# TEAM-AIOLY/OCM-VAE-SIMCA

Hardware: AMD Instinct MI355X
Metric: spectra/sec SIMCA fit+Q/T² score at 1M×2048 (higher is better)
Workload: dtype f32

## Files before the change

### ocm-vae-simca_amd/csrc/ocm_score.hip

```cpp
#include "ocm_internal.h"

#include <utility>

namespace {

constexpr int SW = 4;
constexpr int SR = 32;
constexpr int SROWS = SW * SR;

struct DecArgs {
  int32_t enabled;
  int32_t type;
  double t2_scale, q_scale, dlim;
};

using ocm::dred_of;

template <int KT, int NW>
__device__ __forceinline__ void score_epilogue(double* tls, double* sred, const double (&accT64)[KT][16], double q64,
                                               int64_t row0, int64_t m, int k, int a_diag,
                                               const double* __restrict__ A, float* __restrict__ T_out,
                                               double* T2_out, float* __restrict__ Q_out, DecArgs dec,
                                               double* __restrict__ acc_out, int64_t acc_stride,
                                               double* __restrict__ stat_part, int ldt = 0,
// ... 261 lines not shown
template <int N>
__device__ __forceinline__ void wait_vv(f32x4& h) {
  asm volatile("s_waitcnt vmcnt(%1)" : "+v"(h) : "n"(N));
}
__device__ __forceinline__ float xlane(int src, float v) {
  return __builtin_bit_cast(float, __builtin_amdgcn_ds_bpermute(src, __builtin_bit_cast(int, v)));
}

#ifdef OCM_S1P_DIAG_NOMFMA
#define OCM_MF(ACC, A, B) ""
#define OCM_M4(ACC, A, B) ""
#else
#define OCM_MF(ACC, A, B) "v_mfma_f32_16x16x4_f32 %[" #ACC "], %[" #A "], %[" #B "], %[" #ACC "]\n\t"
#define OCM_M4(ACC, A, B) "v_mfma_f32_4x4x1_16b_f32 %[" #ACC "], %[" #A "], %[" #B "], %[" #ACC "]\n\t"
#endif
template <bool EX>
__device__ __forceinline__ void s1_block(f32x4& acA, f32x4& acB, f32x4& acC, f32x4& acD, f32x4& acE, f32x4& acF,
                                         const f32x4& a, const float (&b)[4], const f32x4& x) {
  if constexpr (EX)
    asm("s_nop 1\n\t" OCM_M4(cE, b0, x0) OCM_MF(cA, a0, x0) OCM_M4(cF, b1, x1) OCM_MF(cB, a1, x1)
            OCM_M4(cE, b2, x2) OCM_MF(cC, a2, x2) OCM_M4(cF, b3, x3) OCM_MF(cD, a3, x3)
        : [cA] "+v"(acA), [cB] "+v"(acB), [cC] "+v"(acC), [cD] "+v"(acD), [cE] "+v"(acE), [cF] "+v"(acF)
        : [a0] "v"(a[0]), [a1] "v"(a[1]), [a2] "v"(a[2]), [a3] "v"(a[3]), [b0] "v"(b[0]), [b1] "v"(b[1]),
          [b2] "v"(b[2]), [b3] "v"(b[3]), [x0] "a"(x[0]), [x1] "a"(x[1]), [x2] "a"(x[2]), [x3] "a"(x[3]));
  else
    asm("s_nop 1\n\t" OCM_MF(cA, a0, x0) OCM_MF(cB, a1, x1) OCM_MF(cC, a2, x2) OCM_MF(cD, a3, x3)
        : [cA] "+v"(acA), [cB] "+v"(acB), [cC] "+v"(acC), [cD] "+v"(acD)
        : [a0] "v"(a[0]), [a1] "v"(a[1]), [a2] "v"(a[2]), [a3] "v"(a[3]), [x0] "a"(x[0]), [x1] "a"(x[1]),
          [x2] "a"(x[2]), [x3] "a"(x[3]));
}

#ifdef OCM_S1P_DIAG_NOMFMA
#define OCM_M2(R, A, T) ""
#else
#define OCM_M2(R, A, T) "v_mfma_f32_16x16x4_f32 %[" #R "], %[" #A "], %[" #T "], %[" #R "]\n\t"
#endif
#define OCM_RD(S, P) "v_accvgpr_read_b32 %[" #S "], %[" #P "]\n\t"
#define OCM_FM(Q, S) "v_fmac_f32_e32 %[" #Q "], %[" #S "], %[" #S "]\n\t"
template <bool EX, bool QW>
__device__ __forceinline__ void s2_pair(f32x4& x0, f32x4& x1, const float (&a0)[5], const float (&a1)[5], float m0,
                                        float m1, const float (&tB)[5], float one, const f32x4& p0, const f32x4& p1,
                                        float (&q)[4]) {
  float s[4];
  if constexpr (EX && QW)
    asm volatile("s_nop 1\n\t" OCM_M4(x0, m0, on) OCM_M4(x1, m1, on) "s_nop 4\n\t" OCM_M2(x0, u0, t0) OCM_M2(x1, w0, t0) OCM_RD(s0, p00) OCM_RD(s1, p10) OCM_RD(s2, p01) OCM_RD(s3, p11) OCM_M2(x0, u1, t1) OCM_FM(q0, s0) OCM_FM(q1, s1) OCM_FM(q2, s2) OCM_FM(q3, s3) OCM_M2(x1, w1, t1) OCM_RD(s0, p02) OCM_RD(s1, p12) OCM_RD(s2, p03) OCM_RD(s3, p13) OCM_M2(x0, u2, t2) OCM_FM(q0, s0) OCM_FM(q1, s1) OCM_FM(q2, s2) OCM_FM(q3, s3) OCM_M2(x1, w2, t2) OCM_M2(x0, u3, t3) OCM_M2(x1, w3, t3) OCM_M2(x0, u4, t4) OCM_M2(x1, w4, t4)
        : [x0] "+a"(x0), [x1] "+a"(x1), [q0] "+v"(q[0]), [q1] "+v"(q[1]), [q2] "+v"(q[2]), [q3] "+v"(q[3]), [s0] "=&v"(s[0]), [s1] "=&v"(s[1]), [s2] "=&v"(s[2]), [s3] "=&v"(s[3])
        : [u0] "v"(a0[0]), [u1] "v"(a0[1]), [u2] "v"(a0[2]), [u3] "v"(a0[3]), [u4] "v"(a0[4]), [w0] "v"(a1[0]), [w1] "v"(a1[1]), [w2] "v"(a1[2]), [w3] "v"(a1[3]), [w4] "v"(a1[4]), [m0] "v"(m0), [m1] "v"(m1), [t0] "v"(tB[0]), [t1] "v"(tB[1]), [t2] "v"(tB[2]), [t3] "v"(tB[3]), [t4] "v"(tB[4]), [on] "v"(one), [p00] "a"(p0[0]), [p01] "a"(p0[1]), [p02] "a"(p0[2]), [p03] "a"(p0[3]), [p10] "a"(p1[0]), [p11] "a"(p1[1]), [p12] "a"(p1[2]), [p13] "a"(p1[3]));
  else if constexpr (EX)
    asm volatile("s_nop 1\n\t" OCM_M4(x0, m0, on) OCM_M4(x1, m1, on) "s_nop 4\n\t" OCM_M2(x0, u0, t0) OCM_M2(x1, w0, t0) OCM_M2(x0, u1, t1) OCM_M2(x1, w1, t1) OCM_M2(x0, u2, t2) OCM_M2(x1, w2, t2) OCM_M2(x0, u3, t3) OCM_M2(x1, w3, t3) OCM_M2(x0, u4, t4) OCM_M2(x1, w4, t4)
        : [x0] "+a"(x0), [x1] "+a"(x1)
        : [u0] "v"(a0[0]), [u1] "v"(a0[1]), [u2] "v"(a0[2]), [u3] "v"(a0[3]), [u4] "v"(a0[4]), [w0] "v"(a1[0]), [w1] "v"(a1[1]), [w2] "v"(a1[2]), [w3] "v"(a1[3]), [w4] "v"(a1[4]), [m0] "v"(m0), [m1] "v"(m1), [t0] "v"(tB[0]), [t1] "v"(tB[1]), [t2] "v"(tB[2]), [t3] "v"(tB[3]), [t4] "v"(tB[4]), [on] "v"(one));
  else if constexpr (QW)
    asm volatile("s_nop 1\n\t" OCM_M4(x0, m0, on) OCM_M4(x1, m1, on) "s_nop 4\n\t" OCM_M2(x0, u0, t0) OCM_M2(x1, w0, t0) OCM_RD(s0, p00) OCM_RD(s1, p10) OCM_RD(s2, p01) OCM_RD(s3, p11) OCM_M2(x0, u1, t1) OCM_FM(q0, s0) OCM_FM(q1, s1) OCM_FM(q2, s2) OCM_FM(q3, s3) OCM_M2(x1, w1, t1) OCM_RD(s0, p02) OCM_RD(s1, p12) OCM_RD(s2, p03) OCM_RD(s3, p13) OCM_M2(x0, u2, t2) OCM_FM(q0, s0) OCM_FM(q1, s1) OCM_FM(q2, s2) OCM_FM(q3, s3) OCM_M2(x1, w2, t2) OCM_M2(x0, u3, t3) OCM_M2(x1, w3, t3)
        : [x0] "+a"(x0), [x1] "+a"(x1), [q0] "+v"(q[0]), [q1] "+v"(q[1]), [q2] "+v"(q[2]), [q3] "+v"(q[3]), [s0] "=&v"(s[0]), [s1] "=&v"(s[1]), [s2] "=&v"(s[2]), [s3] "=&v"(s[3])
        : [u0] "v"(a0[0]), [u1] "v"(a0[1]), [u2] "v"(a0[2]), [u3] "v"(a0[3]), [w0] "v"(a1[0]), [w1] "v"(a1[1]), [w2] "v"(a1[2]), [w3] "v"(a1[3]), [m0] "v"(m0), [m1] "v"(m1), [t0] "v"(tB[0]), [t1] "v"(tB[1]), [t2] "v"(tB[2]), [t3] "v"(tB[3]), [on] "v"(one), [p00] "a"(p0[0]), [p01] "a"(p0[1]), [p02] "a"(p0[2]), [p03] "a"(p0[3]), [p10] "a"(p1[0]), [p11] "a"(p1[1]), [p12] "a"(p1[2]), [p13] "a"(p1[3]));
  else
    asm volatile("s_nop 1\n\t" OCM_M4(x0, m0, on) OCM_M4(x1, m1, on) "s_nop 4\n\t" OCM_M2(x0, u0, t0) OCM_M2(x1, w0, t0) OCM_M2(x0, u1, t1) OCM_M2(x1, w1, t1) OCM_M2(x0, u2, t2) OCM_M2(x1, w2, t2) OCM_M2(x0, u3, t3) OCM_M2(x1, w3, t3)
        : [x0] "+a"(x0), [x1] "+a"(x1)
        : [u0] "v"(a0[0]), [u1] "v"(a0[1]), [u2] "v"(a0[2]), [u3] "v"(a0[3]), [w0] "v"(a1[0]), [w1] "v"(a1[1]), [w2] "v"(a1[2]), [w3] "v"(a1[3]), [m0] "v"(m0), [m1] "v"(m1), [t0] "v"(tB[0]), [t1] "v"(tB[1]), [t2] "v"(tB[2]), [t3] "v"(tB[3]), [on] "v"(one));
  (void)s, (void)p0, (void)p1, (void)q;
}
template <bool EX>
__device__ __forceinline__ void s1_block_v(f32x4& acA, f32x4& acB, f32x4& acC, f32x4& acD, f32x4& acE, f32x4& acF,
                                           const f32x4& a, const float (&b)[4], const f32x4& x) {
  if constexpr (EX)
    asm("s_nop 1\n\t" OCM_M4(cE, b0, x0) OCM_MF(cA, a0, x0) OCM_M4(cF, b1, x1) OCM_MF(cB, a1, x1)
            OCM_M4(cE, b2, x2) OCM_MF(cC, a2, x2) OCM_M4(cF, b3, x3) OCM_MF(cD, a3, x3)
        : [cA] "+v"(acA), [cB] "+v"(acB), [cC] "+v"(acC), [cD] "+v"(acD), [cE] "+v"(acE), [cF] "+v"(acF)
        : [a0] "v"(a[0]), [a1] "v"(a[1]), [a2] "v"(a[2]), [a3] "v"(a[3]), [b0] "v"(b[0]), [b1] "v"(b[1]),
          [b2] "v"(b[2]), [b3] "v"(b[3]), [x0] "v"(x[0]), [x1] "v"(x[1]), [x2] "v"(x[2]), [x3] "v"(x[3]));
  else
    asm("s_nop 1\n\t" OCM_MF(cA, a0, x0) OCM_MF(cB, a1, x1) OCM_MF(cC, a2, x2) OCM_MF(cD, a3, x3)
        : [cA] "+v"(acA), [cB] "+v"(acB), [cC] "+v"(acC), [cD] "+v"(acD)
        : [a0] "v"(a[0]), [a1] "v"(a[1]), [a2] "v"(a[2]), [a3] "v"(a[3]), [x0] "v"(x[0]), [x1] "v"(x[1]),
          [x2] "v"(x[2]), [x3] "v"(x[3]));
}
#undef OCM_MF
#undef OCM_M4
#undef OCM_M2
#undef OCM_RD
#undef OCM_FM
}

#ifdef OCM_S1P_W8
static bool s1p_w8_enabled() {
  const char* v = getenv("OCM_S1P_W8_ON");
  return !v || v[0] != '0';
}
#endif

template <int NJ, bool EX, int HH = -1, int WV = 4>
__global__ __launch_bounds__(64 * WV, 1) void k_score_1p(const float* __restrict__ X, int64_t ldx,
                                                     const int64_t* __restrict__ rows, int64_t m,
                                                     const double* __restrict__ P, const double* __restrict__ mu,
                                                     const double* __restrict__ adiag, int k,
                                                     float* __restrict__ T_out, double* __restrict__ T2_out,
                                                     float* __restrict__ Q_out, DecArgs dec,
                                                     double* __restrict__ acc_out, int64_t acc_stride,
                                                     double* __restrict__ stat_part, int64_t ntiles,
                                                     PrepArgs pa, const float* __restrict__ ptaps,
                                                     const float* __restrict__ prow) {
  using namespace s1p;
  constexpr int W = WV;
  constexpr int NT = 64 * WV;
  constexpr int TPB = WV == 4 ? 2 : 1;
  constexpr bool PREP = HH >= 0;
  constexpr int GL = NJ + (HH > 0 ? 1 : 0);
  constexpr int PW = 16 * NJ;
  constexpr int PP = W * PW;
  constexpr int NCH = PP / 4;
  static_assert(NJ % 4 == 0 && 2 * NJ - 1 <= 63, "64-column wave slices, vmcnt range");
  __shared__ f32x4 P0s[16 * NCH];
  __shared__ float nmuL[PP];
  __shared__ double pmuL[20];
  __shared__ double tpart[TPB][W * 20 * R];
  __shared__ double qpart[2][W * R];
  const int tid = threadIdx.x, lane = tid & 63;
  const int w = __builtin_amdgcn_readfirstlane(tid >> 6);
  const int ln = lane & 15, lq = lane >> 4;

  {
    constexpr int PE = 16 * NCH / NT;
    constexpr int UB = PE < 8 ? PE : 8;
    static_assert(PE % UB == 0, "prologue batches");
#pragma unroll
    for (int i0 = 0; i0 < PE; i0 += UB) {
      double v[UB][4];
#pragma unroll
      for (int u = 0; u < UB; ++u) {
        const int e = tid + (i0 + u) * NT, c = e / NCH, ch = e - c * NCH;
        const double* src = P + (int64_t)(c < k ? c : 0) * PP + 4 * ch;
#pragma unroll
        for (int q = 0; q < 4; ++q) v[u][q] = src[q];
      }
#pragma unroll
      for (int u = 0; u < UB; ++u) {
        const int e = tid + (i0 + u) * NT, c = e / NCH, ch = e - c * NCH;
        f32x4 x;
#pragma unroll
        for (int q = 0; q < 4; ++q) x[q] = c < k ? (float)v[u][q] : 0.f;
        P0s[c * NCH + (ch ^ sw(c))] = x;
      }
    }
    constexpr int ME = PP / NT;
    float nm[ME];
#pragma unroll
    for (int i = 0; i < ME; ++i) nm[i] = -(float)mu[tid + i * NT];
#pragma unroll
    for (int i = 0; i < ME; ++i) nmuL[tid + i * NT] = nm[i];
    constexpr int CL = PP / 64;
    double muv[CL];
#pragma unroll
    for (int i = 0; i < CL; ++i) muv[i] = mu[lane + 64 * i];
    for (int c = w; c < 20; c += W) {
      double s = 0.0;
      if (c < k) {
        double pv[CL];
#pragma unroll
        for (int i = 0; i < CL; ++i) pv[i] = P[(int64_t)c * PP + lane + 64 * i];
#pragma unroll
        for (int i = 0; i < CL; ++i) s += pv[i] * muv[i];
      }
      s = wave_sum_f64(s);
      if (lane == 0) pmuL[c] = s;
    }
  }
  float p1a[EX ? NJ : 1];
  constexpr bool NOP1B = EX && ((NJ == 32 && HH > 4) || WV == 8);
  float p1b[EX && !NOP1B ? NJ : 1];
  if constexpr (EX) {
    const bool p1v = 16 + lq < k;
    const double* p1r = P + (int64_t)(p1v ? 16 + lq : 0) * PP + w * PW;
    double pa_[NJ], pb_[NOP1B ? 1 : NJ];
#pragma unroll
    for (int j = 0; j < NJ; ++j) {
      pa_[j] = p1r[16 * j + ln];
      if constexpr (!NOP1B) pb_[j] = p1r[16 * j + (ln ^ (8 * (lq >> 1)))];
    }
#pragma unroll
    for (int j = 0; j < NJ; ++j) {
      p1a[j] = p1v ? (float)pa_[j] : 0.f;
      if constexpr (!NOP1B) p1b[j] = p1v ? (float)pb_[j] : 0.f;
    }
  }
  __shared__ double adL[WV == 8 ? 20 : 1];
  double ad[WV == 8 ? 1 : 5];
  if constexpr (WV == 8) {
    if (tid < 20) adL[tid] = tid < k ? adiag[tid] : 0.0;
  } else {
#pragma unroll
    for (int s = 0; s < 5; ++s) ad[s] = lq + 4 * s < k ? adiag[lq + 4 * s] : 0.0;
  }
  int b1[4];
#pragma unroll
  for (int b = 0; b < 4; ++b) b1[b] = ln * NCH + w * (PW / 4) + ((4 * b + lq) ^ sw(ln));
  int b2[4][4];
#pragma unroll
  for (int s = 0; s < 4; ++s)
#pragma unroll
    for (int b = 0; b < 4; ++b) {
      const int c = 4 * s + lq;
      b2[s][b] = 4 * (c * NCH + w * (PW / 4) + ((4 * b + (ln >> 2)) ^ sw(c))) + (ln & 3);
    }
  const float* p0f = reinterpret_cast<const float*>(P0s);
  const int bperm = 4 * (16 * (ln & 3) + ((4 * lq) ^ (8 * ((ln & 3) >> 1))));
  const int bpermA = 4 * (16 * (ln & 3) + 4 * lq);
  const float one = 1.f;
  __syncthreads();

  const int64_t G = gridDim.x;
  auto col_base = [&](int64_t row) { return X + row * ldx + w * PW + 4 * lq; };
  auto index_of = [&](int64_t tt) -> int64_t {
    if (!rows) {
      const int64_t r = tt * R + ln;
      return r < m ? r : m - 1;
    }
    int64_t v = 0;
#pragma unroll
    for (int i = 0; i < R; ++i) {
      const int64_t r = tt * R + i;
      const int64_t ri = rows[r < m ? r : m - 1];
      v = ln == i ? ri : v;
    }
    return v;
  };

  f32x4 XA[NJ], XB[NJ];
  double st[4] = {0.0, 0.0, 0.0, 0.0};
  double tt[5];
  float tB[5];
  double T2 = 0.0, T2prev = 0.0;

  float ctap[HH > 0 ? HH + 1 : 1];
  if constexpr (HH > 0)
#pragma unroll
    for (int t = 1; t <= HH; ++t) ctap[t] = ptaps[HH + t];
  auto rowstat_of = [&](int64_t tt, float& mr, float& sr) {
    mr = 0.f;
    sr = 1.f;
    if (!PREP || !pa.snv) return;
#pragma unroll
    for (int i = 0; i < R; ++i) {
      const int64_t r = tt * R + i;
      const int64_t rr = r < m ? r : m - 1;
      const int64_t xi = rows ? rows[rr] : rr;
      const float mi = prow[2 * xi], si = prow[2 * xi + 1];
      mr = ln == i ? mi : mr;
      sr = ln == i ? si : sr;
    }
  };
  auto stencil_e = [&](const float* win, float sr, int e) __attribute__((always_inline)) -> float {
    const int o = (HH > 0 ? HH : 0) + e;
    float a;
    if constexpr (HH <= 0) {
      a = win[o];
    } else {
      a = 0.f;
#pragma unroll
      for (int t = 1; t <= HH; ++t) a = fmaf(ctap[t], __fsub_rn(win[o + t], win[o - t]), a);
    }
    return ocm::mul_nc(a, sr);
  };
  auto stencil = [&](const float* win, float sr) __attribute__((always_inline)) -> f32x4 {
    f32x4 y;
#pragma unroll
    for (int e = 0; e < 4; ++e) y[e] = stencil_e(win, sr, e);
    return y;
  };
  auto edge_fix = [&](f32x4& y, const f32x4& ucur, float sr, bool left) __attribute__((always_inline)) {
    if constexpr (HH > 0) {
      f32x4 q1, q2, q3;
#pragma unroll
      for (int e = 0; e < 4; ++e) {
        q1[e] = xlane(4 * (lane ^ 16), ucur[e]);
        q2[e] = xlane(4 * (lane ^ 32), ucur[e]);
        q3[e] = xlane(4 * (lane ^ 48), ucur[e]);
      }
      float row16[16];
#pragma unroll
      for (int sq = 0; sq < 4; ++sq)
#pragma unroll
        for (int e = 0; e < 4; ++e) {
          const int kk = lq ^ sq;
          row16[4 * sq + e] = kk == 0 ? ucur[e] : kk == 1 ? q1[e] : kk == 2 ? q2[e] : q3[e];
        }
      const int Wn = 2 * HH + 1;
#pragma unroll
      for (int i = 0; i < HH; ++i) {
        const float* et = ptaps + Wn + (left ? i : HH + i) * Wn;
        const int s0 = left ? 0 : 16 - Wn;
        const int cl = left ? i : 16 - HH + i;
        const float ref = row16[cl];
        float a = 0.f;
#pragma unroll
        for (int t = 0; t < Wn; ++t) a = fmaf(et[t], __fsub_rn(row16[s0 + t], ref), a);
        const float yv = ocm::mul_nc(a, sr);
#pragma unroll
        for (int e = 0; e < 4; ++e)
          if (4 * lq + e == cl) y[e] = yv;
      }
    }
  };

  auto exchange = [&](const f32x4& uprev, const f32x4& ucur, const f32x4& unext, float* win)
      __attribute__((always_inline)) {
    constexpr int H_ = HH > 0 ? HH : 0;
    constexpr int NL1 = H_ < 4 ? H_ : 4;
#pragma unroll
    for (int e = 4 - NL1; e < 4; ++e) {
      win[H_ - 4 + e] = xlane(4 * ((lane + 48) & 63), lq == 3 ? uprev[e] : ucur[e]);
      win[H_ + 4 + (e - (4 - NL1))] =
          xlane(4 * ((lane + 16) & 63), lq == 0 ? unext[e - (4 - NL1)] : ucur[e - (4 - NL1)]);
    }
    if constexpr (H_ > 4) {
#pragma unroll
      for (int e = 8 - H_; e < 4; ++e)
        win[H_ - 8 + e] = xlane(4 * (lane ^ 32), lq >= 2 ? uprev[e] : ucur[e]);
#pragma unroll
      for (int e = 0; e < H_ - 4; ++e)
        win[H_ + 8 + e] = xlane(4 * (lane ^ 32), lq <= 1 ? unext[e] : ucur[e]);
    }
#pragma unroll
    for (int e = 0; e < 4; ++e) win[H_ + e] = ucur[e];
  };

  auto sweep1 = [&](f32x4 (&Y)[NJ], f32x4& hy, int buf, int64_t tile, auto XGc) __attribute__((always_inline)) {
    constexpr int XG = decltype(XGc)::value;
    f32x4 acA = {0.f, 0.f, 0.f, 0.f}, acB = acA, acC = acA, acD = acA, acE = acA, acF = acA;
    double t64[4] = {0.0, 0.0, 0.0, 0.0}, x164[4] = {0.0, 0.0, 0.0, 0.0};
    f32x4 aN = P0s[b1[0]];
    float bN[4] = {0.f, 0.f, 0.f, 0.f};
    if constexpr (EX)
#pragma unroll
      for (int e = 0; e < 4; ++e)
        bN[e] = NOP1B ? xlane(bpermA + 4 * e, p1a[0])
                      : __builtin_bit_cast(float, __builtin_amdgcn_ds_bpermute(bperm + 4 * e, __builtin_bit_cast(int, p1b[0])));
    auto operands = [&](auto J, f32x4& a, float (&b)[4]) __attribute__((always_inline)) {
      constexpr int j = decltype(J)::value;
      a = aN;
#pragma unroll
      for (int e = 0; e < 4; ++e) b[e] = bN[e];
      if constexpr (j + 1 < NJ) {
        aN = P0s[b1[(j + 1) & 3] + 16 * ((j + 1) >> 2)];
        if constexpr (EX)
#pragma unroll
          for (int e = 0; e < 4; ++e)
            bN[e] = __builtin_bit_cast(float,
                                       __builtin_amdgcn_ds_bpermute(NOP1B ? bpermA + 4 * e : bperm + 4 * e,
                                                                    __builtin_bit_cast(int, NOP1B ? p1a[j + 1] : p1b[NOP1B ? 0 : j + 1])));
      }
    };
    auto flush = [&]() __attribute__((always_inline)) {
      asm volatile("s_nop 11" : "+v"(acA), "+v"(acB), "+v"(acC), "+v"(acD), "+v"(acE), "+v"(acF));
#pragma unroll
      for (int i = 0; i < 4; ++i) {
        t64[i] += ((double)acA[i] + (double)acB[i]) + ((double)acC[i] + (double)acD[i]);
        x164[i] += (double)acE[i] + (double)acF[i];
        acA[i] = acB[i] = acC[i] = acD[i] = acE[i] = acF[i] = 0.f;
      }
    };
    if constexpr (!PREP) {
      static_for<NJ>([&](auto J) {
        constexpr int j = decltype(J)::value;
        f32x4 a;
        float b[4];
        operands(J, a, b);
        wait_vm<NJ - 1 - j + XG>(Y[j]);
        s1_block<EX>(acA, acB, acC, acD, acE, acF, a, b, Y[j]);
        __builtin_amdgcn_sched_barrier(0);
        if constexpr ((j & 15) == 15 || j == NJ - 1) {
          flush();
        }
      });
    } else {
      constexpr int H_ = HH > 0 ? HH : 0;
      float win[4 + 2 * H_];
      float mr, sr;
      rowstat_of(tile, mr, sr);
      constexpr int W0 = NJ - 3 + XG < 63 ? NJ - 3 + XG : 63;
      wait_vm<W0>(Y[2]);
      wait_vm<W0>(Y[1]);
      wait_vm<W0>(Y[0]);
      wait_vv<W0>(hy);
      auto raw = [&](const f32x4& v) __attribute__((always_inline)) {
        f32x4 u = v;
        if constexpr (HH == 0)
#pragma unroll
          for (int e = 0; e < 4; ++e) u[e] = __fsub_rn(u[e], mr);
        return u;
      };
      f32x4 uprev = raw(hy), ucur = raw(Y[0]), unext = raw(Y[1]);
      f32x4 yE = {0.f, 0.f, 0.f, 0.f};
      if constexpr (HH > 0) {
        wait_vm<XG>(Y[NJ - 1]);
        if (w == 0) edge_fix(yE, ucur, sr, true);
        if (w == W - 1) edge_fix(yE, raw(Y[NJ - 1]), sr, false);
      }
      auto patch = [&](f32x4& y, bool right) __attribute__((always_inline)) {
        if constexpr (HH > 0)
#pragma unroll
          for (int e = 0; e < 4; ++e) {
            const int cl = 4 * lq + e;
            const bool ed = right ? (w == W - 1) & (cl >= 16 - HH) : (w == 0) & (cl < HH);
            y[e] = ed ? yE[e] : y[e];
          }
      };
      auto advance = [&](const f32x4& nx) __attribute__((always_inline)) {
        unext = raw(nx);
        exchange(uprev, ucur, unext, win);
        uprev = ucur;
        ucur = unext;
      };
      exchange(uprev, ucur, unext, win);
      uprev = ucur;
      ucur = unext;
      f32x4 y = stencil(win, sr);
      patch(y, false);
      if constexpr (NJ == 1) patch(y, true);
      advance(Y[2]);
      static_for<NJ>([&](auto J) {
        constexpr int j = decltype(J)::value;
        f32x4 a;
        float b[4];
        operands(J, a, b);
        f32x4 yn = y;
#pragma unroll
        for (int e = 0; e < 4; ++e) {
          if constexpr (EX)
            (e & 1 ? acF : acE) = __builtin_amdgcn_mfma_f32_4x4x1f32(b[e], y[e], e & 1 ? acF : acE, 0, 0, 0);
          f32x4& c = e == 0 ? acA : e == 1 ? acB : e == 2 ? acC : acD;
          c = __builtin_amdgcn_mfma_f32_16x16x4f32(a[e], y[e], c, 0, 0, 0);
          if constexpr (j + 1 < NJ) yn[e] = stencil_e(win, sr, e);
        }
        asm volatile("" : "=a"(Y[j]) : "0"(y));
        if constexpr (j + 1 < NJ) {
          y = yn;
          if constexpr (j + 1 == NJ - 1) patch(y, true);
          if constexpr (j + 2 < NJ) {
            if constexpr (j + 3 < NJ) {
              wait_vm<NJ - 4 - j + XG>(Y[j + 3]);
              advance(Y[j + 3]);
            } else {
              advance(hy);
            }
          }
        }
        __builtin_amdgcn_sched_barrier(0);
        if constexpr ((j & 15) == 15 || j == NJ - 1) {
          flush();
        }
      });
    }
    if constexpr (TPB == 1) {
      asm volatile("s_waitcnt lgkmcnt(0)" ::: "memory");
      __builtin_amdgcn_s_barrier();
      asm volatile("" ::: "memory");
    }
    double* tp = tpart[TPB == 1 ? 0 : buf];
#pragma unroll
    for (int i = 0; i < 4; ++i) tp[(w * 20 + 4 * lq + i) * R + ln] = t64[i];
    if constexpr (EX) {
#pragma unroll
      for (int u = 0; u < 4; ++u) {
        x164[u] += __shfl_xor(x164[u], 16, 64);
        x164[u] += __shfl_xor(x164[u], 32, 64);
      }
      if (lq == 0)
#pragma unroll
        for (int u = 0; u < 4; ++u) tp[(w * 20 + 16 + u) * R + ln] = x164[u];
    }
  };
  auto compute_t = [&](int64_t t, int buf) {
    const double* tp = tpart[TPB == 1 ? 0 : buf];
#pragma unroll
    for (int s = 0; s < 5; ++s) {
      double v = 0.0;
      if (s < 4 || EX) {
#pragma unroll
        for (int ww = 0; ww < W; ++ww) v += tp[(ww * 20 + lq + 4 * s) * R + ln];
        v -= pmuL[lq + 4 * s];
      }
      tt[s] = v;
    }
    T2 = 0.0;
#pragma unroll
    for (int s = 0; s < 5; ++s) T2 += tt[s] * tt[s] * (WV == 8 ? adL[lq + 4 * s] : ad[s < (WV == 8 ? 1 : 5) ? s : 0]);
    T2 += __shfl_xor(T2, 16, 64);
    T2 += __shfl_xor(T2, 32, 64);
    const int64_t row = t * R + ln;
    if (T_out && w == 0 && row < m)
#pragma unroll
      for (int s = 0; s < 5; ++s)
        if (lq + 4 * s < k) T_out[row * k + lq + 4 * s] = (float)tt[s];
#pragma unroll
    for (int s = 0; s < 5; ++s) tB[s] = -(float)tt[s];
  };
  auto halo_ptr = [&](const float* pre) -> const float* {
    const bool left = lq >= 2;
    return left ? (w > 0 ? pre - 16 : pre) : (w < W - 1 ? pre + 16 * NJ : pre);
  };
  auto sweep2 = [&](f32x4 (&Z)[NJ], f32x4& hz, const float* pre, int buf) __attribute__((always_inline)) {
    if constexpr (HH > 0) load_v(hz, halo_ptr(pre));
    float q[4] = {0.f, 0.f, 0.f, 0.f};
    double q64 = 0.0;
    float aN[2][5], mN[2];
    auto read_a = [&](auto J, float (&dst)[5], float& mdst) {
      constexpr int j = decltype(J)::value;
#pragma unroll
      for (int s = 0; s < 4; ++s) dst[s] = p0f[b2[s][j & 3] + 64 * (j >> 2)];
      dst[4] = EX ? p1a[j] : 0.f;
      mdst = nmuL[w * PW + 16 * j + 4 * lq + (ln & 3)];
    };
    read_a(std::integral_constant<int, 0>{}, aN[0], mN[0]);
    read_a(std::integral_constant<int, 1>{}, aN[1], mN[1]);
    static_for<NJ / 2>([&](auto H) {
      constexpr int j = 2 * decltype(H)::value;
      float a0[5], a1[5];
#pragma unroll
      for (int s = 0; s < 5; ++s) {
        a0[s] = aN[0][s];
        a1[s] = aN[1][s];
      }
      const float m0 = mN[0], m1 = mN[1];
      if constexpr (j + 2 < NJ) {
        read_a(std::integral_constant<int, j + 2>{}, aN[0], mN[0]);
        read_a(std::integral_constant<int, j + 3>{}, aN[1], mN[1]);
      }
      if constexpr (j == 0) {
        s2_pair<EX, false>(Z[0], Z[1], a0, a1, m0, m1, tB, one, Z[0], Z[1], q);
      } else {
        s2_pair<EX, true>(Z[j], Z[j + 1], a0, a1, m0, m1, tB, one, Z[j - 2], Z[j - 1], q);
        __builtin_amdgcn_sched_barrier(0);
        refill_a<64 * (j - 2)>(Z[j - 2], pre);
        refill_a<64 * (j - 1)>(Z[j - 1], pre);
        if constexpr (((j - 2) & 15) == 14) {
          q64 += ((double)q[0] + (double)q[1]) + ((double)q[2] + (double)q[3]);
          q[0] = q[1] = q[2] = q[3] = 0.f;
        }
      }
      __builtin_amdgcn_sched_barrier(0);
    });
    asm volatile("s_nop 11" : "+a"(Z[NJ - 2]), "+a"(Z[NJ - 1]));
#pragma unroll
    for (int e = 0; e < 4; ++e) {
      q[e & 1] = fmaf(Z[NJ - 2][e], Z[NJ - 2][e], q[e & 1]);
      q[2 + (e & 1)] = fmaf(Z[NJ - 1][e], Z[NJ - 1][e], q[2 + (e & 1)]);
    }
    __builtin_amdgcn_sched_barrier(0);
    refill_a<64 * (NJ - 2)>(Z[NJ - 2], pre);
    refill_a<64 * (NJ - 1)>(Z[NJ - 1], pre);
    q64 += ((double)q[0] + (double)q[1]) + ((double)q[2] + (double)q[3]);
    q64 += __shfl_xor(q64, 16, 64);
    q64 += __shfl_xor(q64, 32, 64);
    if (lq == 0) qpart[buf][w * R + ln] = q64;
  };
  auto finish = [&](int64_t t, int buf) {
    double Q = 0.0;
#pragma unroll
    for (int ww = 0; ww < W; ++ww) Q += qpart[buf][ww * R + ln];
    const int64_t row = t * R + ln;
    if (w == 0 && lq == 0 && row < m) {
      const float Qf = (float)Q;
      if (T2_out) T2_out[row] = T2prev;
      if (Q_out) Q_out[row] = Qf;
      if (dec.enabled) {
        const double dr = ocm::dred_of(dec.type, T2prev * dec.t2_scale, (double)Qf * dec.q_scale);
        acc_out[row * acc_stride] = dr < dec.dlim ? 1.0 : 0.0;
      }
      st[0] += T2prev;
      st[1] += T2prev * T2prev;
      st[2] += (double)Qf;
      st[3] += (double)Qf * (double)Qf;
    }
  };
  auto lds_barrier = [&]() {
    asm volatile("s_waitcnt lgkmcnt(0)" ::: "memory");
    __builtin_amdgcn_s_barrier();
    asm volatile("" ::: "memory");
  };

  int64_t t = blockIdx.x;
  auto clamp_tile = [&](int64_t tt) { return tt < ntiles ? tt : t; };
  f32x4 hA = {0.f, 0.f, 0.f, 0.f}, hB = hA;
  {
    const float* p0 = col_base(index_of(t));
    if constexpr (HH > 0) load_v(hA, halo_ptr(p0));
    static_for<NJ>([&](auto J) { load_a<64 * decltype(J)::value>(XA[decltype(J)::value], p0); });
  }
  sweep1(XA, hA, 0, t, std::integral_constant<int, 0>{});
  {
    const float* p1 = col_base(index_of(clamp_tile(t + G)));
    if constexpr (HH > 0) load_v(hB, halo_ptr(p1));
    static_for<NJ>([&](auto J) { load_a<64 * decltype(J)::value>(XB[decltype(J)::value], p1); });
  }
  lds_barrier();
  compute_t(t, 0);
  int buf = 0;
#ifdef OCM_S1P_STAMPS
  double cyc[4] = {0.0, 0.0, 0.0, 0.0};
  uint64_t c_last = __builtin_readcyclecounter();
#define OCM_STAMP(I)                                    \
  {                                                     \
    const uint64_t c_now = __builtin_readcyclecounter(); \
    cyc[I] += (double)(c_now - c_last);                  \
    c_last = c_now;                                      \
  }
#else
#define OCM_STAMP(I)
#endif
  auto step = [&](f32x4 (&Xc)[NJ], f32x4& hc, f32x4 (&Yn)[NJ], f32x4& hn) __attribute__((always_inline)) -> bool {
    const int64_t tn = t + G;
    const bool more = tn < ntiles;
    OCM_STAMP(3)
    sweep2(Xc, hc, col_base(index_of(clamp_tile(tn + G))), buf);
    OCM_STAMP(0)
    if (more || PREP) sweep1(Yn, hn, buf ^ 1, tn, std::integral_constant<int, GL>{});
    OCM_STAMP(1)
    lds_barrier();
    OCM_STAMP(2)
    T2prev = T2;
    finish(t, buf);
    if (!more) return false;
    t = tn;
    buf ^= 1;
    compute_t(t, buf);
    return true;
  };
#undef OCM_STAMP
  for (;;) {
    if (!step(XA, hA, XB, hB)) break;
    if (!step(XB, hB, XA, hA)) break;
  }
#pragma unroll
  for (int j = 0; j < NJ; ++j) {
    wait_vm<0>(XA[j]);
    wait_vm<0>(XB[j]);
  }
  if constexpr (HH > 0) {
    wait_vv<0>(hA);
    wait_vv<0>(hB);
  }
#ifdef OCM_S1P_STAMPS
#pragma unroll
  for (int i = 0; i < 4; ++i) st[i] = cyc[i] / 64.0;
#endif
  if (stat_part) {
#pragma unroll
    for (int i = 0; i < 4; ++i) st[i] = wave_sum_f64(st[i]);
    if (w == 0 && lane == 0)
#pragma unroll
      for (int i = 0; i < 4; ++i) stat_part[(int64_t)blockIdx.x * 4 + i] = st[i];
  }
}

__global__ __launch_bounds__(1024) void k_stats_reduce(const double* __restrict__ part, int64_t nblk,
                                                       double* __restrict__ out) {
  __shared__ double red[16];
  const int w = threadIdx.x >> 6, lane = threadIdx.x & 63;
  const int col = w & 3, sl = w >> 2;
  double v0 = 0.0, v1 = 0.0, v2 = 0.0, v3 = 0.0;
  int64_t i = (int64_t)sl * 64 + lane;
  for (; i + 3 * 256 < nblk; i += 4 * 256) {
    v0 += part[i * 4 + col];
    v1 += part[(i + 256) * 4 + col];
    v2 += part[(i + 512) * 4 + col];
    v3 += part[(i + 768) * 4 + col];
  }
  for (; i < nblk; i += 256) v0 += part[i * 4 + col];
  double v = wave_sum_f64((v0 + v1) + (v2 + v3));
  if (lane == 0) red[w] = v;
  __syncthreads();
  if (threadIdx.x < 4) out[threadIdx.x] = (red[threadIdx.x] + red[4 + threadIdx.x]) + (red[8 + threadIdx.x] + red[12 + threadIdx.x]);
}

__global__ void k_decide(const double* __restrict__ T2, const float* __restrict__ Q, int64_t m, DecArgs dec,
                         double* __restrict__ t2red, double* __restrict__ qred, double* __restrict__ dred,
                         double* __restrict__ acc, int64_t acc_stride) {
  const int64_t i = (int64_t)blockIdx.x * blockDim.x + threadIdx.x;
  if (i >= m) return;
  const double t = T2[i] * dec.t2_scale;
  const double q = (double)Q[i] * dec.q_scale;
  if (t2red) t2red[i] = t;
  if (qred) qred[i] = q;
  const double d = dred_of(dec.type, t, q);
  if (dred) dred[i] = d;
  if (acc) acc[i * acc_stride] = d < dec.dlim ? 1.0 : 0.0;
}

__global__ __launch_bounds__(256) void k_rowsq(const float* __restrict__ x, int64_t ldx, const float* __restrict__ xh,
                                               int64_t ldxh, int64_t m, int p, float* __restrict__ q) {
  const int64_t r = (int64_t)blockIdx.x * 4 + (threadIdx.x >> 6);
  const int lane = threadIdx.x & 63;
  if (r >= m) return;
  double s = 0.0;
  for (int j = lane; j < p; j += 64) {
    const double d = (double)x[r * ldx + j] - (double)xh[r * ldxh + j];
    s += d * d;
  }
  s = wave_sum_f64(s);
  if (lane == 0) q[r] = (float)s;
}

__global__ __launch_bounds__(256) void k_rowsq_minmax(const float* __restrict__ x, int64_t ldx,
                                                      const float* __restrict__ xh, int64_t ldxh, int64_t m, int p,
                                                      float eps, float* __restrict__ q) {
  const int64_t r = (int64_t)blockIdx.x * 4 + (threadIdx.x >> 6);
  const int lane = threadIdx.x & 63;
  if (r >= m) return;
  const float* xr = x + r * ldx;
  const float* hr = xh + r * ldxh;
  float lo = INFINITY, hi = -INFINITY;
  for (int j = lane; j < p; j += 64) {
    const float v = xr[j];
    lo = fminf(lo, v);
    hi = fmaxf(hi, v);
  }
#pragma unroll
  for (int o = 32; o > 0; o >>= 1) {
    lo = fminf(lo, __shfl_xor(lo, o, 64));
    hi = fmaxf(hi, __shfl_xor(hi, o, 64));
  }
  const float den = (hi - lo) + eps;
  double s = 0.0;
  for (int j = lane; j < p; j += 64) {
    const float a = fminf(fmaxf((xr[j] - lo) / den, 0.f), 1.f);
    const float b = fminf(fmaxf((hr[j] - lo) / den, 0.f), 1.f);
    const float d = a - b;
    s += (double)(d * d);
  }
  s = wave_sum_f64(s);
  if (lane == 0) q[r] = (float)s;
}

__global__ void k_cast_f64_f32(const double* __restrict__ a, int64_t n, float* __restrict__ b) {
// ... 68 lines not shown
#undef OCM_SCORE_LAUNCH
    OCM_CHECK_LAUNCH("k_score");
  }
  if (stats_out) {
    hipLaunchKernelGGL(k_stats_reduce, dim3(1), dim3(1024), 0, st, part, nblk, stats_out);
    OCM_CHECK_LAUNCH("k_stats_reduce");
  }
  return OCM_OK;
}

}

extern "C" {

int ocm_score_f32(ocm_ctx* ctx, const float* X, int64_t ldx, const int64_t* rows, int64_t m, int32_t p,
                  const double* P, const double* mu, const double* A, int32_t k, float* T_out, double* T2_out,
                  float* Q_out, const ocm_decision* dec, double* accept_out, int64_t accept_stride,
                  double* stats_out, void* stream) {
  OCM_REQUIRE(ctx && X && P && mu && A, "ocm_score_f32: NULL argument");
  OCM_REQUIRE(m >= 0 && p > 0 && ldx >= p, "ocm_score_f32: bad shape");
  OCM_REQUIRE(k >= 1 && k <= 64, "ocm_score_f32: 1 <= k <= 64 (larger k: ocm_score_f32_diag)");
  OCM_REQUIRE(!dec || accept_out, "ocm_score_f32: decision requires accept_out");
  return score_direct(ctx, X, ldx, rows, m, p, P, mu, A, 0, k, T_out, T2_out, Q_out, dec, accept_out,
                      accept_stride, stats_out, (hipStream_t)stream);
}

}

namespace {

int score_diag_impl(ocm_ctx* ctx, const float* X, int64_t ldx, const int64_t* rows, int64_t m, int32_t p,
                    const PrepArgs* pp, const double* P, const double* mu, const double* a_diag, int32_t k,
                    float* T_out, double* T2_out, float* Q_out, const ocm_decision* dec, double* accept_out,
                    int64_t accept_stride, double* stats_out, hipStream_t st) {
  int nj = p / 64;
  const bool vec = (ldx % 4 == 0) && ((reinterpret_cast<uintptr_t>(X) & 15) == 0);
  bool one_pass = vec && p % 64 == 0 && (nj == 4 || nj == 8 || nj == 16 || nj == 32) && k <= 20;
  const PrepArgs pa = pp ? *pp : PrepArgs{};
  if (pp && !pa.fused_form()) one_pass = false;
  if (!one_pass && pp) {
    if (m == 0) {
      if (stats_out) OCM_HIP(hipMemsetAsync(stats_out, 0, 4 * sizeof(double), st));
      return OCM_OK;
    }
    float* Y = nullptr;
    OCM_HIP(hipMallocAsync(reinterpret_cast<void**>(&Y), (size_t)m * p * sizeof(float), st));
    ++ctx->prep_materialised;
    int rc = ocm::prep_apply(ctx, X, ldx, rows, m, p, pa, Y, p, st);
    if (rc == OCM_OK)
      rc = score_diag_impl(ctx, Y, p, nullptr, m, p, nullptr, P, mu, a_diag, k, T_out, T2_out, Q_out, dec,
                           accept_out, accept_stride, stats_out, st);
    const hipError_t e = hipFreeAsync(Y, st);
    if (rc == OCM_OK && e != hipSuccess) return ocm::fail(OCM_ERR_HIP, std::string("hipFreeAsync: ") + hipGetErrorString(e));
    return rc;
  }
  if (!one_pass)
    return score_direct(ctx, X, ldx, rows, m, p, P, mu, a_diag, 1, k, T_out, T2_out, Q_out, dec, accept_out,
                        accept_stride, stats_out, st);
  if (m == 0) {
    if (stats_out) OCM_HIP(hipMemsetAsync(stats_out, 0, 4 * sizeof(double), st));
    return OCM_OK;
  }
  const int64_t ntiles = (m + s1p::R - 1) / s1p::R;
  const int grid = (int)std::min<int64_t>(ctx->num_cus, ntiles);
  double* part = nullptr;
  if (stats_out) {
    void* wsp = ocm::workspace(ctx, (size_t)grid * 4 * sizeof(double) + 256, st);
    if (!wsp) return OCM_ERR_NOMEM;
    part = static_cast<double*>(wsp);
  }
  DecArgs d{};
  if (dec) {
    d.enabled = 1;
    d.type = dec->type;
    d.t2_scale = dec->t2_scale;
    d.q_scale = dec->q_scale;
    d.dlim = dec->dlim;
  }
  {
    ocm::TimedRegion tr(ctx, OCM_KERNEL_SCORE, st);
#define OCM_S1P_H(NJ_, EX_, H_)                                                                                 \
  hipLaunchKernelGGL((k_score_1p<NJ_, EX_, H_>), dim3(grid), dim3(256), 0, st, X, ldx, rows, m, P, mu, a_diag, k, \
                     T_out, T2_out, Q_out, d, accept_out, accept_stride, part, ntiles, pa, pa.taps, pa.rowstat)
#ifdef OCM_S1P_W8
    if (nj == 32 && !pp && s1p_w8_enabled()) {
      if (k > 16)
        hipLaunchKernelGGL((k_score_1p<16, true, -1, 8>), dim3(grid), dim3(512), 0, st, X, ldx, rows, m, P, mu, a_diag,
                           k, T_out, T2_out, Q_out, d, accept_out, accept_stride, part, ntiles, pa, pa.taps,
                           pa.rowstat);
      else
        hipLaunchKernelGGL((k_score_1p<16, false, -1, 8>), dim3(grid), dim3(512), 0, st, X, ldx, rows, m, P, mu,
                           a_diag, k, T_out, T2_out, Q_out, d, accept_out, accept_stride, part, ntiles, pa, pa.taps,
                           pa.rowstat);
      nj = 0;
    }
#endif
#define OCM_S1P(NJ_, EX_)                                  \
  if (!pp)                                                 \
    OCM_S1P_H(NJ_, EX_, -1);                               \
  else if (pa.h == 0)                                      \
    OCM_S1P_H(NJ_, EX_, 0);                                \
  else if (pa.h == 2)                                      \
    OCM_S1P_H(NJ_, EX_, 2);                                \
  else                                                     \
    OCM_S1P_H(NJ_, EX_, 7);
#define OCM_S1P_K(NJ_) \
  if (k > 16) {        \
    OCM_S1P(NJ_, true) \
  } else {             \
    OCM_S1P(NJ_, false) \
  }
    if (nj == 0) {
    } else if (nj == 32) {
      OCM_S1P_K(32)
    } else if (nj == 16) {
      OCM_S1P_K(16)
    } else if (nj == 8) {
      OCM_S1P_K(8)
    } else {
      OCM_S1P_K(4)
    }
#undef OCM_S1P_K
#undef OCM_S1P
#undef OCM_S1P_H
  }
  OCM_CHECK_LAUNCH("k_score_1p");
  if (stats_out) {
    hipLaunchKernelGGL(k_stats_reduce, dim3(1), dim3(1024), 0, st, part, (int64_t)grid, stats_out);
    OCM_CHECK_LAUNCH("k_stats_reduce");
  }
  return OCM_OK;
}

}

extern "C" {

int ocm_score_f32_diag(ocm_ctx* ctx, const float* X, int64_t ldx, const int64_t* rows, int64_t m, int32_t p,
                       const double* P, const double* mu, const double* a_diag, int32_t k, float* T_out,
                       double* T2_out, float* Q_out, const ocm_decision* dec, double* accept_out,
                       int64_t accept_stride, double* stats_out, void* stream) {
  OCM_REQUIRE(ctx && X && P && mu && a_diag, "ocm_score_f32_diag: NULL argument");
  OCM_REQUIRE(m >= 0 && p > 0 && ldx >= p, "ocm_score_f32_diag: bad shape");
  OCM_REQUIRE(k >= 1 && k <= p, "ocm_score_f32_diag: 1 <= k <= p");
  OCM_REQUIRE(!dec || accept_out, "ocm_score_f32_diag: decision requires accept_out");
  return score_diag_impl(ctx, X, ldx, rows, m, p, nullptr, P, mu, a_diag, k, T_out, T2_out, Q_out, dec, accept_out,
                         accept_stride, stats_out, (hipStream_t)stream);
}

int ocm_score_f32_diag_prep(ocm_ctx* ctx, const float* X, int64_t ldx, const int64_t* rows, int64_t m, int32_t p,
                            const ocm_prep* prep, const double* P, const double* mu, const double* a_diag, int32_t k,
                            float* T_out, double* T2_out, float* Q_out, const ocm_decision* dec,
                            double* accept_out, int64_t accept_stride, double* stats_out, void* stream) {
  OCM_REQUIRE(ctx && X && P && mu && a_diag, "ocm_score_f32_diag_prep: NULL argument");
  OCM_REQUIRE(m >= 0 && p > 0 && ldx >= p, "ocm_score_f32_diag_prep: bad shape");
  OCM_REQUIRE(k >= 1 && k <= p, "ocm_score_f32_diag_prep: 1 <= k <= p");
  OCM_REQUIRE(!dec || accept_out, "ocm_score_f32_diag_prep: decision requires accept_out");
  if (int rc = ocm::check_prep(prep, p, "ocm_score_f32_diag_prep")) return rc;
  const PrepArgs pa = ocm::prep_args(prep);
  return score_diag_impl(ctx, X, ldx, rows, m, p, &pa, P, mu, a_diag, k, T_out, T2_out, Q_out, dec, accept_out,
                         accept_stride, stats_out, (hipStream_t)stream);
}

int ocm_decide(ocm_ctx* ctx, const double* T2, const float* Q, int64_t m, const ocm_decision* dec, double* t2red_out,
               double* qred_out, double* dred_out, double* accept_out, int64_t accept_stride, void* stream) {
  OCM_REQUIRE(ctx && T2 && Q && dec, "ocm_decide: NULL argument");
  if (m <= 0) return OCM_OK;
  DecArgs d{1, dec->type, dec->t2_scale, dec->q_scale, dec->dlim};
  hipLaunchKernelGGL(k_decide, dim3((unsigned)((m + 255) / 256)), dim3(256), 0, (hipStream_t)stream, T2, Q, m, d,
                     t2red_out, qred_out, dred_out, accept_out, accept_stride);
  OCM_CHECK_LAUNCH("k_decide");
  return OCM_OK;
}

int ocm_rowsq_residual_f32(ocm_ctx* ctx, const float* x, int64_t ldx, const float* xhat, int64_t ldxh, int64_t m,
                           int32_t p, float* q_out, void* stream) {
  OCM_REQUIRE(ctx && x && xhat && q_out, "ocm_rowsq_residual_f32: NULL argument");
  OCM_REQUIRE(p > 0 && ldx >= p && (ldxh == 0 || ldxh >= p), "ocm_rowsq_residual_f32: bad shape");
  if (m <= 0) return OCM_OK;
// ... 27 lines not shown
```

Before: 57.07 million.

## Add phased 8-wave score kernel with two wave groups interleaving tiles

Replaces the experimental 8-wave variant with a 'phased' kernel in which two groups of 4 waves each process alternating tiles over the full 2048-column slice (NJ=32). One group computes sweep1 while the other runs sweep2, with staggered barriers. Per-group LDS buffers hold the T partials, and running stats are accumulated in LDS. Register pressure is reduced by dropping XB double-buffering, recomputing LDS offsets via XOR, and using bpermute shuffles. It is enabled by default when k>16 with plain rows. The intent is to overlap the two phases across SIMDs and raise latency hiding, at the cost of losing the per-wave double-buffered prefetch.

```diff
diff --git a/ocm-vae-simca_amd/csrc/ocm_score.hip b/ocm-vae-simca_amd/csrc/ocm_score.hip
--- a/ocm-vae-simca_amd/csrc/ocm_score.hip
+++ b/ocm-vae-simca_amd/csrc/ocm_score.hip
@@ -367,9 +367,9 @@
 #undef OCM_FM
 }
 
-#ifdef OCM_S1P_W8
-static bool s1p_w8_enabled() {
-  const char* v = getenv("OCM_S1P_W8_ON");
+#ifdef OCM_EXP_SELECTORS
+static bool s1p_phased_enabled() {
+  const char* v = getenv("OCM_S1P_PHASED_ON");
   return !v || v[0] != '0';
 }
 #endif
@@ -386,9 +386,9 @@
                                                      PrepArgs pa, const float* __restrict__ ptaps,
                                                      const float* __restrict__ prow) {
   using namespace s1p;
-  constexpr int W = WV;
+  static_assert(WV == 4 || (WV == 8 && HH < 0), "phased kernel: plain rows");
+  constexpr int W = 4;
   constexpr int NT = 64 * WV;
-  constexpr int TPB = WV == 4 ? 2 : 1;
   constexpr bool PREP = HH >= 0;
   constexpr int GL = NJ + (HH > 0 ? 1 : 0);
   constexpr int PW = 16 * NJ;
@@ -398,11 +398,15 @@
   __shared__ f32x4 P0s[16 * NCH];
   __shared__ float nmuL[PP];
   __shared__ double pmuL[20];
-  __shared__ double tpart[TPB][W * 20 * R];
+  __shared__ double tpart[2][W * 20 * R];
   __shared__ double qpart[2][W * R];
-  const int tid = threadIdx.x, lane = tid & 63;
-  const int w = __builtin_amdgcn_readfirstlane(tid >> 6);
-  const int ln = lane & 15, lq = lane >> 4;
+  const int wv = __builtin_amdgcn_readfirstlane((int)threadIdx.x >> 6);
+  const int lane = WV == 8 ? (int)__lane_id() : (int)threadIdx.x & 63;
+  const int tid = WV == 8 ? 64 * wv + lane : (int)threadIdx.x;
+  const int w = wv & 3;
+  const int g = wv >> 2;
+  int ln = lane & 15, lq = lane >> 4;
+  if constexpr (WV == 8) asm volatile("" : "+v"(ln), "+v"(lq));
 
   {
     constexpr int PE = 16 * NCH / NT;
@@ -426,6 +430,7 @@
         for (int q = 0; q < 4; ++q) x[q] = c < k ? (float)v[u][q] : 0.f;
         P0s[c * NCH + (ch ^ sw(c))] = x;
       }
+      if constexpr (WV == 8) __builtin_amdgcn_sched_barrier(0);
     }
     constexpr int ME = PP / NT;
     float nm[ME];
@@ -434,10 +439,30 @@
 #pragma unroll
     for (int i = 0; i < ME; ++i) nmuL[tid + i * NT] = nm[i];
     constexpr int CL = PP / 64;
+    if constexpr (WV == 8) {
+      for (int c = wv; c < 20; c += WV) {
+        double s = 0.0;
+        if (c < k) {
+#pragma unroll
+          for (int i0 = 0; i0 < CL; i0 += 8) {
+            double pv[8], mv[8];
+#pragma unroll
+            for (int i = 0; i < 8; ++i) {
+              pv[i] = P[(int64_t)c * PP + lane + 64 * (i0 + i)];
+              mv[i] = mu[lane + 64 * (i0 + i)];
+            }
+#pragma unroll
+            for (int i = 0; i < 8; ++i) s += pv[i] * mv[i];
+          }
+        }
+        s = wave_sum_f64(s);
+        if (lane == 0) pmuL[c] = s;
+      }
+    } else {
     double muv[CL];
 #pragma unroll
     for (int i = 0; i < CL; ++i) muv[i] = mu[lane + 64 * i];
-    for (int c = w; c < 20; c += W) {
+    for (int c = wv; c < 20; c += WV) {
       double s = 0.0;
       if (c < k) {
         double pv[CL];
@@ -448,6 +473,7 @@
       }
       s = wave_sum_f64(s);
       if (lane == 0) pmuL[c] = s;
+    }
     }
   }
   float p1a[EX ? NJ : 1];
@@ -456,40 +482,63 @@
   if constexpr (EX) {
     const bool p1v = 16 + lq < k;
     const double* p1r = P + (int64_t)(p1v ? 16 + lq : 0) * PP + w * PW;
-    double pa_[NJ], pb_[NOP1B ? 1 : NJ];
-#pragma unroll
-    for (int j = 0; j < NJ; ++j) {
-      pa_[j] = p1r[16 * j + ln];
-      if constexpr (!NOP1B) pb_[j] = p1r[16 * j + (ln ^ (8 * (lq >> 1)))];
-    }
-#pragma unroll
-    for (int j = 0; j < NJ; ++j) {
-      p1a[j] = p1v ? (float)pa_[j] : 0.f;
-      if constexpr (!NOP1B) p1b[j] = p1v ? (float)pb_[j] : 0.f;
+    constexpr int PB = WV == 8 ? 8 : NJ;
+#pragma unroll
+    for (int j0 = 0; j0 < NJ; j0 += PB) {
+      double pa_[PB], pb_[NOP1B ? 1 : PB];
+#pragma unroll
+      for (int j = 0; j < PB; ++j) {
+        pa_[j] = p1r[16 * (j0 + j) + ln];
+        if constexpr (!NOP1B) pb_[j] = p1r[16 * (j0 + j) + (ln ^ (8 * (lq >> 1)))];
+      }
+#pragma unroll
+      for (int j = 0; j < PB; ++j) {
+        p1a[j0 + j] = p1v ? (float)pa_[j] : 0.f;
+        if constexpr (!NOP1B) p1b[j0 + j] = p1v ? (float)pb_[j] : 0.f;
+      }
     }
   }
   __shared__ double adL[WV == 8 ? 20 : 1];
   double ad[WV == 8 ? 1 : 5];
+  __shared__ double stL[WV == 8 ? 2 * 4 * R : 1];
   if constexpr (WV == 8) {
     if (tid < 20) adL[tid] = tid < k ? adiag[tid] : 0.0;
+    if (tid < 2 * 4 * R) stL[tid] = 0.0;
   } else {
 #pragma unroll
     for (int s = 0; s < 5; ++s) ad[s] = lq + 4 * s < k ? adiag[lq + 4 * s] : 0.0;
   }
-  int b1[4];
-#pragma unroll
-  for (int b = 0; b < 4; ++b) b1[b] = ln * NCH + w * (PW / 4) + ((4 * b + lq) ^ sw(ln));
-  int b2[4][4];
+  constexpr int NB = WV == 8 ? 1 : 4;
+  int b1[NB];
+#pragma unroll
+  for (int b = 0; b < NB; ++b) b1[b] = ln * NCH + w * (PW / 4) + ((4 * b + lq) ^ sw(ln));
+  int b2[4][NB];
 #pragma unroll
   for (int s = 0; s < 4; ++s)
 #pragma unroll
-    for (int b = 0; b < 4; ++b) {
+    for (int b = 0; b < NB; ++b) {
       const int c = 4 * s + lq;
       b2[s][b] = 4 * (c * NCH + w * (PW / 4) + ((4 * b + (ln >> 2)) ^ sw(c))) + (ln & 3);
     }
+  auto B1 = [&](int b) { return WV == 8 ? b1[0] ^ (4 * b) : b1[b & (NB - 1)]; };
+  auto B2 = [&](int s, int b) { return WV == 8 ? b2[s][0] ^ (16 * b) : b2[s][b & (NB - 1)]; };
   const float* p0f = reinterpret_cast<const float*>(P0s);
   const int bperm = 4 * (16 * (ln & 3) + ((4 * lq) ^ (8 * ((ln & 3) >> 1))));
-  const int bpermA = 4 * (16 * (ln & 3) + 4 * lq);
+  int bpermA = 4 * (16 * (ln & 3) + 4 * lq);
+  auto fresh = [&](int& v) __attribute__((always_inline)) {
+    if constexpr (WV == 8) asm volatile("" : "+v"(v));
+  };
+  auto shx = [&](double v, int o) __attribute__((always_inline)) -> double {
+    if constexpr (WV == 8) {
+      const int a = 4 * ((16 * lq + ln) ^ o);
+      const uint64_t u = __builtin_bit_cast(uint64_t, v);
+      const uint32_t lo = __builtin_amdgcn_ds_bpermute(a, (int)(uint32_t)u);
+      const uint32_t hi = __builtin_amdgcn_ds_bpermute(a, (int)(uint32_t)(u >> 32));
+      return __builtin_bit_cast(double, ((uint64_t)hi << 32) | lo);
+    } else {
+      return __shfl_xor(v, o, 64);
+    }
+  };
   const float one = 1.f;
   __syncthreads();
 
@@ -510,7 +559,7 @@
     return v;
   };
 
-  f32x4 XA[NJ], XB[NJ];
+  f32x4 XA[NJ], XB[WV == 8 ? 1 : NJ];
   double st[4] = {0.0, 0.0, 0.0, 0.0};
   double tt[5];
   float tB[5];
@@ -611,9 +660,10 @@
 
   auto sweep1 = [&](f32x4 (&Y)[NJ], f32x4& hy, int buf, int64_t tile, auto XGc) __attribute__((always_inline)) {
     constexpr int XG = decltype(XGc)::value;
+    fresh(ln), fresh(lq), fresh(b1[0]), fresh(bpermA);
     f32x4 acA = {0.f, 0.f, 0.f, 0.f}, acB = acA, acC = acA, acD = acA, acE = acA, acF = acA;
     double t64[4] = {0.0, 0.0, 0.0, 0.0}, x164[4] = {0.0, 0.0, 0.0, 0.0};
-    f32x4 aN = P0s[b1[0]];
+    f32x4 aN = P0s[B1(0)];
     float bN[4] = {0.f, 0.f, 0.f, 0.f};
     if constexpr (EX)
 #pragma unroll
@@ -626,7 +676,7 @@
 #pragma unroll
       for (int e = 0; e < 4; ++e) b[e] = bN[e];
       if constexpr (j + 1 < NJ) {
-        aN = P0s[b1[(j + 1) & 3] + 16 * ((j + 1) >> 2)];
+        aN = P0s[B1((j + 1) & 3) + 16 * ((j + 1) >> 2)];
         if constexpr (EX)
 #pragma unroll
           for (int e = 0; e < 4; ++e)
@@ -736,19 +786,14 @@
         }
       });
     }
-    if constexpr (TPB == 1) {
-      asm volatile("s_waitcnt lgkmcnt(0)" ::: "memory");
-      __builtin_amdgcn_s_barrier();
-      asm volatile("" ::: "memory");
-    }
-    double* tp = tpart[TPB == 1 ? 0 : buf];
+    double* tp = tpart[buf];
 #pragma unroll
     for (int i = 0; i < 4; ++i) tp[(w * 20 + 4 * lq + i) * R + ln] = t64[i];
     if constexpr (EX) {
 #pragma unroll
       for (int u = 0; u < 4; ++u) {
-        x164[u] += __shfl_xor(x164[u], 16, 64);
-        x164[u] += __shfl_xor(x164[u], 32, 64);
+        x164[u] += shx(x164[u], 16);
+        x164[u] += shx(x164[u], 32);
       }
       if (lq == 0)
 #pragma unroll
@@ -756,7 +801,7 @@
     }
   };
   auto compute_t = [&](int64_t t, int buf) {
-    const double* tp = tpart[TPB == 1 ? 0 : buf];
+    const double* tp = tpart[buf];
 #pragma unroll
     for (int s = 0; s < 5; ++s) {
       double v = 0.0;
@@ -770,8 +815,8 @@
     T2 = 0.0;
 #pragma unroll
     for (int s = 0; s < 5; ++s) T2 += tt[s] * tt[s] * (WV == 8 ? adL[lq + 4 * s] : ad[s < (WV == 8 ? 1 : 5) ? s : 0]);
-    T2 += __shfl_xor(T2, 16, 64);
-    T2 += __shfl_xor(T2, 32, 64);
+    T2 += shx(T2, 16);
+    T2 += shx(T2, 32);
     const int64_t row = t * R + ln;
     if (T_out && w == 0 && row < m)
 #pragma unroll
@@ -786,13 +831,14 @@
   };
   auto sweep2 = [&](f32x4 (&Z)[NJ], f32x4& hz, const float* pre, int buf) __attribute__((always_inline)) {
     if constexpr (HH > 0) load_v(hz, halo_ptr(pre));
+    fresh(ln), fresh(lq), fresh(b2[0][0]), fresh(b2[1][0]), fresh(b2[2][0]), fresh(b2[3][0]);
     float q[4] = {0.f, 0.f, 0.f, 0.f};
     double q64 = 0.0;
     float aN[2][5], mN[2];
     auto read_a = [&](auto J, float (&dst)[5], float& mdst) {
       constexpr int j = decltype(J)::value;
 #pragma unroll
-      for (int s = 0; s < 4; ++s) dst[s] = p0f[b2[s][j & 3] + 64 * (j >> 2)];
+      for (int s = 0; s < 4; ++s) dst[s] = p0f[B2(s, j & 3) + 64 * (j >> 2)];
       dst[4] = EX ? p1a[j] : 0.f;
       mdst = nmuL[w * PW + 16 * j + 4 * lq + (ln & 3)];
     };
@@ -835,8 +881,8 @@
     refill_a<64 * (NJ - 2)>(Z[NJ - 2], pre);
     refill_a<64 * (NJ - 1)>(Z[NJ - 1], pre);
     q64 += ((double)q[0] + (double)q[1]) + ((double)q[2] + (double)q[3]);
-    q64 += __shfl_xor(q64, 16, 64);
-    q64 += __shfl_xor(q64, 32, 64);
+    q64 += shx(q64, 16);
+    q64 += shx(q64, 32);
     if (lq == 0) qpart[buf][w * R + ln] = q64;
   };
   auto finish = [&](int64_t t, int buf) {
@@ -852,10 +898,18 @@
         const double dr = ocm::dred_of(dec.type, T2prev * dec.t2_scale, (double)Qf * dec.q_scale);
         acc_out[row * acc_stride] = dr < dec.dlim ? 1.0 : 0.0;
       }
-      st[0] += T2prev;
-      st[1] += T2prev * T2prev;
-      st[2] += (double)Qf;
-      st[3] += (double)Qf * (double)Qf;
+      if constexpr (WV == 8) {
+        double* sp = stL + g * 4 * R + ln;
+        sp[0] += T2prev;
+        sp[R] += T2prev * T2prev;
+        sp[2 * R] += (double)Qf;
+        sp[3 * R] += (double)Qf * (double)Qf;
+      } else {
+        st[0] += T2prev;
+        st[1] += T2prev * T2prev;
+        st[2] += (double)Qf;
+        st[3] += (double)Qf * (double)Qf;
+      }
     }
   };
   auto lds_barrier = [&]() {
@@ -867,6 +921,68 @@
   int64_t t = blockIdx.x;
   auto clamp_tile = [&](int64_t tt) { return tt < ntiles ? tt : t; };
   f32x4 hA = {0.f, 0.f, 0.f, 0.f}, hB = hA;
+  if constexpr (WV == 8) {
+    const int64_t b = blockIdx.x;
+    const int64_t npos = (ntiles - b + G - 1) / G;
+    const int64_t NP = (npos + 1) / 2;
+    auto tile_at = [&](int64_t n) { return b + (2 * n + g) * G; };
+    auto load_tile = [&](int64_t tl) { return tl < ntiles ? tl : b; };
+    {
+      const float* p0 = col_base(index_of(load_tile(tile_at(0))));
+      static_for<NJ>([&](auto J) { load_a<64 * decltype(J)::value>(XA[decltype(J)::value], p0); });
+    }
+    if (g == 1) lds_barrier();
+    for (int64_t n = 0; n < NP; ++n) {
+      const int64_t tl = tile_at(n);
+      if (n > 0) {
+        T2prev = T2;
+        finish(tl - 2 * G, g);
+      }
+      sweep1(XA, hA, g, load_tile(tl), std::integral_constant<int, 0>{});
+      lds_barrier();
+      compute_t(tl, g);
+      sweep2(XA, hA, col_base(index_of(load_tile(tile_at(n + 1)))), g);
+      lds_barrier();
+    }
+    T2prev = T2;
+    finish(tile_at(NP - 1), g);
+    if (g == 0) lds_barrier();
+#pragma unroll
+    for (int j = 0; j < NJ; ++j) wait_vm<0>(XA[j]);
+#ifdef OCM_S1P_HWID
+    if (stat_part) {
+      __shared__ int hwL[8];
+      const int simd = __builtin_amdgcn_s_getreg(4 | (4 << 6) | (1 << 11));
+      if (ln == 0 && lq == 0) hwL[wv] = simd;
+      lds_barrier();
+      if (wv == 0 && ln == 0 && lq == 0) {
+        int diff = 0;
+        for (int i = 0; i < 4; ++i) diff += hwL[i] != hwL[i + 4];
+        stat_part[b * 4 + 0] = diff;
+        stat_part[b * 4 + 1] = hwL[0];
+        stat_part[b * 4 + 2] = hwL[1];
+        stat_part[b * 4 + 3] = hwL[5];
+      }
+    }
+    return;
+#endif
+    if (stat_part) {
+      lds_barrier();
+      if (wv == 0) {
+#pragma unroll
+        for (int i = 0; i < 4; ++i) {
+          double s0 = 0.0, s1 = 0.0;
+#pragma unroll
+          for (int r = 0; r < R; ++r) {
+            s0 += stL[i * R + r];
+            s1 += stL[(4 + i) * R + r];
+          }
+          if (ln == 0 && lq == 0) stat_part[b * 4 + i] = s0 + s1;
+        }
+      }
+    }
+    return;
+  } else {
   {
     const float* p0 = col_base(index_of(t));
     if constexpr (HH > 0) load_v(hA, halo_ptr(p0));
@@ -935,6 +1051,7 @@
     if (w == 0 && lane == 0)
 #pragma unroll
       for (int i = 0; i < 4; ++i) stat_part[(int64_t)blockIdx.x * 4 + i] = st[i];
+  }
   }
 }
 
@@ -1169,19 +1286,24 @@
 #define OCM_S1P_H(NJ_, EX_, H_)                                                                                 \
   hipLaunchKernelGGL((k_score_1p<NJ_, EX_, H_>), dim3(grid), dim3(256), 0, st, X, ldx, rows, m, P, mu, a_diag, k, \
                      T_out, T2_out, Q_out, d, accept_out, accept_stride, part, ntiles, pa, pa.taps, pa.rowstat)
-#ifdef OCM_S1P_W8
-    if (nj == 32 && !pp && s1p_w8_enabled()) {
+#ifdef OCM_EXP_SELECTORS
+    const bool phased = nj == 32 && !pp && s1p_phased_enabled();
+#else
+    const bool phased = nj == 32 && !pp && k > 16;
+#endif
+    if (phased) {
       if (k > 16)
-        hipLaunchKernelGGL((k_score_1p<16, true, -1, 8>), dim3(grid), dim3(512), 0, st, X, ldx, rows, m, P, mu, a_diag,
+        hipLaunchKernelGGL((k_score_1p<32, true, -1, 8>), dim3(grid), dim3(512), 0, st, X, ldx, rows, m, P, mu, a_diag,
                            k, T_out, T2_out, Q_out, d, accept_out, accept_stride, part, ntiles, pa, pa.taps,
                            pa.rowstat);
+#ifdef OCM_EXP_SELECTORS
       else
-        hipLaunchKernelGGL((k_score_1p<16, false, -1, 8>), dim3(grid), dim3(512), 0, st, X, ldx, rows, m, P, mu,
+        hipLaunchKernelGGL((k_score_1p<32, false, -1, 8>), dim3(grid), dim3(512), 0, st, X, ldx, rows, m, P, mu,
                            a_diag, k, T_out, T2_out, Q_out, d, accept_out, accept_stride, part, ntiles, pa, pa.taps,
                            pa.rowstat);
+#endif
       nj = 0;
     }
-#endif
 #define OCM_S1P(NJ_, EX_)                                  \
   if (!pp)                                                 \
     OCM_S1P_H(NJ_, EX_, -1);                               \
```

Result: faster. 58.05 million, median of 6 (+1.7%).
